# DannielSilva/MM-VQA

Measured on AMD Instinct MI355X. Metric: samples/sec ROCO-MLM pretrain (resnet152+transformer, bs16/GPU, 224^2, seq32), higher is better.
Workload: dtype f32; 1 GPU; pretrain/roco_train.py MLM-only: resnet152 + transformer(4 layers, 12 heads), num_vis 5, hidden 768, vocab 30522, per-GPU batch 16, 224x224, T=32; fwd + log_softmax/NLL + bwd + grad all-reduce + Adam; dropout on, train-mode BN; random-init weights; global_batch=16, seq_len=32, parallelism=dp1

## Files before the change

### mm-vqa_amd/csrc/common.h

```cpp
#pragma once
#include <hip/hip_runtime.h>
#include <stdint.h>
#include "../../include/mmvqa.h"

typedef float f32x4 __attribute__((ext_vector_type(4)));
typedef float f32x16 __attribute__((ext_vector_type(16)));

enum { ACT_NONE = 0, ACT_RELU = 1, ACT_GELU = 2, ACT_SERF = 3, ACT_SILU = 4, ACT_SIGMOID = 5 };
enum { PRO_NONE = 0, PRO_AFFINE_RELU = 1, PRO_DZ = 2, PRO_AFFINE = 3, PRO_AFFINE_SILU = 4, PRO_SILU_GATE = 5 };
enum { EPI_PLAIN = 0, EPI_TAP_FWD = 1, EPI_TAP_BWD = 2 };
enum { KIND_FWD = 0, KIND_DGRAD = 1, KIND_WGRAD = 2 };


typedef mmvqa_gemm_desc GemmParams;
typedef mmvqa_attn_desc AttnParams;

__device__ __forceinline__ float erf_pos(float s) {
  float t = 1.0f + s * (0.0705230784f + s * (0.0422820123f + s * (0.0092705272f +
            s * (0.0001520143f + s * (0.0002765672f + s * 0.0000430638f)))));
  t = t * t; t = t * t; t = t * t; t = t * t;
  const float big = 1.0f - 1.0f / t;
  const float s2 = s * s;
  float pl = -7.5757575757e-4f;
  pl = pl * s2 + 4.6296296296e-3f;
  pl = pl * s2 - 2.3809523810e-2f;
  pl = pl * s2 + 0.1f;
// ... 180 lines not shown
```

### mm-vqa_amd/csrc/elementwise.hip

```cpp
#include <cstring>

#include "common.h"

static inline int cdiv_i(long a, long b) { return (int)((a + b - 1) / b); }

static_assert(MMVQA_STAT_SLOTS == 16, "one lane per statistics replica");
__device__ __forceinline__ void stat_fold16(const double* __restrict__ stat, int C, int c, bool live, double& s0,
                                            double& s1) {
  typedef double f64x2 __attribute__((ext_vector_type(2)));
  const int sl = threadIdx.x & 15;
  f64x2 v = {0.0, 0.0};
  if (live) v = *reinterpret_cast<const f64x2*>(stat + ((size_t)sl * C + c) * 2);
  s0 = v[0]; s1 = v[1];
#pragma unroll
  for (int o = 8; o > 0; o >>= 1) { s0 += __shfl_xor(s0, o, 64); s1 += __shfl_xor(s1, o, 64); }
}
__global__ __launch_bounds__(256) void bn_coef_fwd_kernel(const double* __restrict__ stat, int C, double count, float eps,
                                   const float* __restrict__ gamma, const float* __restrict__ beta,
                                   float* __restrict__ run_mean, float* __restrict__ run_var,
                                   long long* __restrict__ nbt, double keep, int reps, int training,
                                   float* __restrict__ scale, float* __restrict__ shift,
                                   float* __restrict__ mean_out, float* __restrict__ invstd_out) {
  const int c = blockIdx.x * 16 + (threadIdx.x >> 4);
  if (blockIdx.x == 0 && threadIdx.x == 0 && training && nbt) *nbt += reps;
// ... 161 lines not shown
    double a[8] = {0, 0, 0, 0, 0, 0, 0, 0};
    for (int t = tid; t < 256; t += C4)
#pragma unroll
      for (int j = 0; j < 8; ++j) a[j] += red[t * 8 + j];
    int slot = blockIdx.x & (MMVQA_STAT_SLOTS - 1);
#pragma unroll
    for (int j = 0; j < 4; ++j) {
      double* d = stat + ((size_t)slot * C + tid * 4 + j) * 2;
      atomicAdd(d, a[j]);
      atomicAdd(d + 1, a[4 + j]);
    }
  }
}

#define LN_MAXV 4
__global__ void layernorm_fwd_kernel(const float* __restrict__ x, const float* __restrict__ res,
                                     const float* __restrict__ gamma, const float* __restrict__ beta,
                                     float* __restrict__ y, float* __restrict__ sum_out,
                                     float* __restrict__ mean_out, float* __restrict__ rstd_out,
                                     int rows, int H, float eps) {
  const int lane = threadIdx.x & 63;
  const int row = blockIdx.x * (blockDim.x >> 6) + (threadIdx.x >> 6);
  if (row >= rows) return;
  const int H4 = H / 4;
  f32x4 v[LN_MAXV];
  float s = 0.f;
#pragma unroll
  for (int j = 0; j < LN_MAXV; ++j) {
    int q = lane + 64 * j;
    v[j] = f32x4{0, 0, 0, 0};
// ... 21 lines not shown
  float rstd = 1.0f / sqrtf(var + eps);
#pragma unroll
  for (int j = 0; j < LN_MAXV; ++j) {
    int q = lane + 64 * j;
    if (q < H4) {
      f32x4 g = reinterpret_cast<const f32x4*>(gamma)[q], b = reinterpret_cast<const f32x4*>(beta)[q], o;
#pragma unroll
      for (int e = 0; e < 4; ++e) o[e] = (v[j][e] - mean) * rstd * g[e] + b[e];
      reinterpret_cast<f32x4*>(y + (size_t)row * H)[q] = o;
    }
  }
  if (lane == 0) { mean_out[row] = mean; rstd_out[row] = rstd; }
}

__global__ void layernorm_bwd_kernel(const float* __restrict__ dy, const float* __restrict__ x,
                                     const float* __restrict__ gamma, const float* __restrict__ mean,
                                     const float* __restrict__ rstd, const float* __restrict__ dres,
                                     float* __restrict__ dx, float* __restrict__ dgamma,
                                     float* __restrict__ dbeta, int rows, int H, int rows_per_wave) {
  extern __shared__ float lds[];
  const int lane = threadIdx.x & 63, wave = threadIdx.x >> 6, nw = blockDim.x >> 6;
  const int H4 = H / 4;
  for (int i = threadIdx.x; i < 2 * H; i += blockDim.x) lds[i] = 0.f;
  __syncthreads();
  f32x4 ag[LN_MAXV], ab[LN_MAXV];
#pragma unroll
  for (int j = 0; j < LN_MAXV; ++j) { ag[j] = f32x4{0, 0, 0, 0}; ab[j] = f32x4{0, 0, 0, 0}; }
  const int row0 = (blockIdx.x * nw + wave) * rows_per_wave;
  for (int rr = 0; rr < rows_per_wave; ++rr) {
    const int row = row0 + rr;
// ... 743 lines not shown
  }
  for (; i < n4; i += stride) {
    f32x4 p0 = P4[i], g0 = G4[i], m0 = M4[i], v0 = V4[i];
    upd(p0, g0, m0, v0);
    P4[i] = p0; M4[i] = m0; V4[i] = v0;
    if (zero_grad) G4[i] = zero;
  }
}

__global__ void axpy_kernel(float* __restrict__ y, const float* __restrict__ x, float a, long n) {
  long i = (long)blockIdx.x * blockDim.x + threadIdx.x;
  long stride = (long)gridDim.x * blockDim.x;
  for (; i < n; i += stride) y[i] += a * x[i];
}

__global__ void colsum_kernel(const float* __restrict__ x, int ld, int rows, int cols, float* __restrict__ out) {
  int c = blockIdx.x * blockDim.x + threadIdx.x;
  if (c >= cols) return;
  int r0 = blockIdx.y * 64, r1 = min(rows, r0 + 64);
  float s = 0.f;
  for (int r = r0; r < r1; ++r) s += x[(size_t)r * ld + c];
  atomicAdd(&out[c], s);
}

__global__ void dropout_kernel(float* __restrict__ x, long n, float p, uint32_t seed) {
  long i = (long)blockIdx.x * blockDim.x + threadIdx.x;
  long stride = (long)gridDim.x * blockDim.x;
  const float ks = 1.0f / (1.0f - p);
  for (; i < n; i += stride) x[i] = (rng_uniform(seed, (uint32_t)i) >= p) ? x[i] * ks : 0.f;
}

// ... 145 lines not shown
  return MMVQA_OK;
}

int k_layernorm_fwd(hipStream_t st, const float* x, const float* res, const float* gamma, const float* beta,
                    float* y, float* sum_out, float* mean, float* rstd, int rows, int H, float eps) {
  if (H % 4 != 0 || H > 256 * LN_MAXV) return mmvqa_set_error(MMVQA_ERR_ARG, "layernorm: H=%d unsupported", H);
  hipLaunchKernelGGL(layernorm_fwd_kernel, dim3(cdiv_i(rows, 4)), dim3(256), 0, st, x, res, gamma, beta, y,
                     sum_out, mean, rstd, rows, H, eps);
  KERNEL_CHECK_RET();
  return MMVQA_OK;
}

int k_layernorm_bwd(hipStream_t st, const float* dy, const float* x, const float* gamma, const float* mean,
                    const float* rstd, const float* dres, float* dx, float* dgamma, float* dbeta, int rows, int H) {
  if (H % 4 != 0 || H > 256 * LN_MAXV) return mmvqa_set_error(MMVQA_ERR_ARG, "layernorm: H=%d unsupported", H);
  int rpw = rows >= 2048 ? 4 : (rows >= 512 ? 2 : 1);
  int grid = cdiv_i(rows, 4 * rpw);
  hipLaunchKernelGGL(layernorm_bwd_kernel, dim3(grid), dim3(256), 2 * H * sizeof(float), st, dy, x, gamma, mean,
                     rstd, dres, dx, dgamma, dbeta, rows, H, rpw);
  KERNEL_CHECK_RET();
  return MMVQA_OK;
}

int k_embed_fwd(hipStream_t st, const long long* ids, const long long* seg, const float* word, const float* pos,
                const float* type, const float* gamma, const float* beta, const float* vis, float* out,
                float* xhat, float* rstd, int B, int T, int H, int num_vis, float eps, float drop_p,
                uint32_t seed) {
  if (H % 4 != 0 || H > 256 * LN_MAXV) return mmvqa_set_error(MMVQA_ERR_ARG, "embed: H=%d unsupported", H);
  hipLaunchKernelGGL(embed_fwd_kernel, dim3(cdiv_i((long)B * T, 4)), dim3(256), 0, st, ids, seg, word, pos, type,
                     gamma, beta, vis, out, xhat, rstd, B, T, H, num_vis, eps, drop_p, seed);
  KERNEL_CHECK_RET();
  return MMVQA_OK;
}

// ... 140 lines not shown
  hipLaunchKernelGGL(adam_kernel<U_>, dim3(grid_for(n / 4, 256, cap > 0 ? cap : 16384)), dim3(256), 0, st, p, g, m, v, n / 4, \
                     (float)(lr / bc1), (float)b1, (float)(1.0 - b1), (float)b2, (float)(1.0 - b2), (float)eps,            \
                     (float)sqrt(bc2), gscale, zero_grad)
  if (unroll >= 4) ADAM_GO(4); else if (unroll == 3) ADAM_GO(3); else if (unroll == 1) ADAM_GO(1); else ADAM_GO(2);
#undef ADAM_GO
  KERNEL_CHECK_RET();
  return MMVQA_OK;
}

int k_axpy(hipStream_t st, float* y, const float* x, float a, long n) {
  hipLaunchKernelGGL(axpy_kernel, dim3(grid_for(n)), dim3(256), 0, st, y, x, a, n);
  KERNEL_CHECK_RET();
  return MMVQA_OK;
}

int k_colsum(hipStream_t st, const float* x, int ld, int rows, int cols, float* out) {
  hipLaunchKernelGGL(colsum_kernel, dim3(cdiv_i(cols, 256), cdiv_i(rows, 64)), dim3(256), 0, st, x, ld, rows, cols,
                     out);
  KERNEL_CHECK_RET();
  return MMVQA_OK;
}

int k_dropout(hipStream_t st, float* x, long n, float p, uint32_t seed) {
  hipLaunchKernelGGL(dropout_kernel, dim3(grid_for(n)), dim3(256), 0, st, x, n, p, seed);
  KERNEL_CHECK_RET();
  return MMVQA_OK;
}

__global__ void pixmask_kernel(int* out, int total, int OH, int OW, int SH, int SW, int KH, int KW, int stride, int pad) {
  const int m = blockIdx.x * blockDim.x + threadIdx.x;
  if (m >= total) return;
  const int rem = m % (OH * OW), oy = rem / OW, ox = rem - oy * OW;
  const int y0 = oy * stride - pad, x0 = ox * stride - pad;
  unsigned mk = 0;
  for (int kh = 0; kh < KH; ++kh)
    for (int kw = 0; kw < KW; ++kw)
      if ((unsigned)(y0 + kh) < (unsigned)SH && (unsigned)(x0 + kw) < (unsigned)SW) mk |= 1u << (kh * KW + kw);
  out[m] = (int)mk;
}

int k_pixmask(hipStream_t st, int* out, int N, int OH, int OW, int SH, int SW, int KH, int KW, int stride, int pad) {
  if (KH * KW > 32) return mmvqa_set_error(MMVQA_ERR_ARG, "pixmask: at most 32 taps");
  const int total = N * OH * OW;
  if (total <= 0) return MMVQA_OK;
  hipLaunchKernelGGL(pixmask_kernel, dim3((total + 255) / 256), dim3(256), 0, st, out, total, OH, OW, SH, SW, KH, KW, stride, pad);
  KERNEL_CHECK_RET();
  return MMVQA_OK;
}

int k_dropout_copy(hipStream_t st, const float* x, float* y, long n, float p, uint32_t seed) {
  hipLaunchKernelGGL(dropout_copy_kernel, dim3(grid_for(n)), dim3(256), 0, st, x, y, n, p, seed);
  KERNEL_CHECK_RET();
  return MMVQA_OK;
}


__global__ void bn_act_add_kernel(const float* __restrict__ z, const float* __restrict__ s,
// ... 645 lines not shown
```

### mm-vqa_amd/csrc/engine.cpp

```cpp
#include "engine.h"

#include <cmath>
#include <cstdarg>
#include <cstdio>
#include <cstring>

static thread_local char g_err[1024] = "";
int mmvqa_set_error(int code, const char* fmt, ...) {
  va_list ap;
  va_start(ap, fmt);
  vsnprintf(g_err, sizeof(g_err), fmt, ap);
  va_end(ap);
  return code;
}
const char* mmvqa_get_error() { return g_err; }

#define TRY(x)                    \
  do {                            \
    int _r = (x);                 \
    if (_r != MMVQA_OK) return _r; \
  } while (0)

namespace {

// ... 211 lines not shown
  if (forced == 1 || forced == 2 || forced == 4 || forced == 8 || forced == 16) return forced;
  const double row_tiles = rows / 64.0;
  return row_tiles >= 32.0 ? 4 : (row_tiles >= 8.0 ? 2 : 1);
}

void plan_bn(Arena& a, BNRef& bn, double count) {
  bn.count = count;
  const size_t C = bn.C;
  bn.scale = a.f(C); bn.shift = a.f(C); bn.mean = a.f(C); bn.invstd = a.f(C);
  bn.P = a.f(C); bn.Q = a.f(C); bn.R = a.f(C);
}

}

static inline int conv_out(int x, int k, int s, int p) { return (x + 2 * p - k) / s + 1; }

size_t engine_plan(mmvqa_engine* e, int B, int T, int IH, int IW) {
  const mmvqa_model_desc& d = e->d;
  if (B <= 0 || T <= 0 || T > 128 || T > d.max_pos || T <= d.num_vis) {
    mmvqa_set_error(MMVQA_ERR_ARG, "plan: bad B=%d T=%d (max_pos %d, num_vis %d, T<=128)", B, T, d.max_pos, d.num_vis);
    return 0;
  }
  e->B = B; e->T = T; e->IH = IH; e->IW = IW;
  e->pixmask_off.clear(); e->ws_ready = false;
  Arena a;
  const int H = d.hidden;
  const size_t M = (size_t)B * T;
  size_t max_io = 0, max_mid = 0, max_tapM = 0;
  if (d.cnn == 1) {
    auto same = [](int in, int k, int s2, int* out) {
// ... 55 lines not shown
  e->SH = conv_out(IH, 7, 2, 3); e->SW = conv_out(IW, 7, 2, 3);
  e->PH = conv_out(e->SH, 3, 2, 1); e->PW = conv_out(e->SW, 3, 2, 1);
  const int w = d.resnet_width;
  const size_t M0 = (size_t)B * e->SH * e->SW;
  e->z0 = a.f(M0 * w);
  plan_bn(a, e->stem_bn, (double)M0);
  e->p0 = a.f((size_t)B * e->PH * e->PW * w);
  e->pool_idx = a.f(((size_t)B * e->PH * e->PW * w + 3) / 4);
  int h = e->PH, wd = e->PW;
  max_io = M0 * w; max_tapM = M0;
  for (auto& blk : e->blocks) {
    blk.N = B; blk.H = h; blk.W = wd;
    blk.OH = conv_out(h, 3, blk.c2.stride, 1); blk.OW = conv_out(wd, 3, blk.c2.stride, 1);
    const size_t Min = (size_t)B * h * wd, Mout = (size_t)B * blk.OH * blk.OW;
    blk.z1 = a.f(Min * blk.c1.Cout);
    if (blk.c2.stride == 1) {
      char key[96];
      snprintf(key, sizeof(key), "%d,%d,%d,%d,%d", B, blk.OH, blk.OW, blk.c2.KH, blk.c2.pad);
      if (!e->pixmask_off.count(key))
        e->pixmask_off[key] = mmvqa_engine::PixGeom{B, blk.OH, blk.OW, h, wd, blk.c2.KH, blk.c2.stride, blk.c2.pad, a.f(Mout)};
    }
    blk.z2 = a.f(Mout * blk.c2.Cout);
    blk.z3 = a.f(Mout * blk.c3.Cout);
    blk.out = a.f(Mout * blk.c3.Cout);
    plan_bn(a, blk.b1, (double)Min);
    plan_bn(a, blk.b2, (double)Mout);
    plan_bn(a, blk.b3, (double)Mout);
    if (blk.has_ds) { blk.zd = a.f(Mout * blk.cd.Cout); plan_bn(a, blk.bd, (double)Mout); }
    if (e->bn_fold) {
      blk.b1.slots = fold_slots((double)Min);
      blk.b2.slots = blk.b3.slots = blk.bd.slots = fold_slots((double)Mout);
    }
    max_io = std::max(max_io, std::max(Min * blk.c1.Cin, Mout * blk.c3.Cout));
    max_mid = std::max(max_mid, std::max(Min * blk.c1.Cout, Mout * blk.c2.Cout));
    h = blk.OH; wd = blk.OW;
  }
// ... 272 lines not shown
}

static int conv_wgrad(mmvqa_engine* e, hipStream_t st, const ConvRef& c, const float* G, const float* z,
                      const BNRef& bn_out, const float* x, const BNRef* bn_in, int N, int H, int W, int OH, int OW) {
  GemmParams g;
  memset(&g, 0, sizeof(g));
  g.M = c.Cout; g.N = c.KH * c.KH * c.Cin; g.K = N * OH * OW;
  g.A = G; g.A2 = z; g.a_ld = c.Cout; g.a_pro = PRO_DZ;
  g.a_c0 = WS(bn_out.P); g.a_c1 = WS(bn_out.Q); g.a_c2 = WS(bn_out.R);
  if (folding(e)) set_fold_bwd(e, g.a_fold, bn_out, false);
  g.B = x; g.b_ld = c.Cin;
  if (bn_in) { g.b_pro = PRO_AFFINE_RELU; g.b_c0 = WS(bn_in->scale); g.b_c1 = WS(bn_in->shift); }
  g.g_SH = H; g.g_SW = W; g.g_Cs = c.Cin; g.g_OH = OH; g.g_OW = OW;
  conv_geom(g, c, H, W, OH, OW);
  g.C = GRD(c.w); g.c_ld = g.N; g.c_atomic = 1;
  if (c.KH > 1 && c.stride == 1 && OH == H && OW == W) {
    char key[96];
    snprintf(key, sizeof(key), "%d,%d,%d,%d,%d", N, OH, OW, c.KH, c.pad);
    auto it = e->pixmask_off.find(key);
    if (it != e->pixmask_off.end()) g.pixmask = reinterpret_cast<int*>(WS(it->second.off));
  }
  RUN(PROF_IGEMM, 2.0 * (double)g.M * g.N * g.K, mmvqa_launch_igemm(g, KIND_WGRAD, 0, 0, st));
  return MMVQA_OK;
}

static int conv_dgrad(mmvqa_engine* e, hipStream_t st, const ConvRef& c, const float* G, const float* z,
                      const BNRef& bn_out, int N, int H, int W, int OH, int OW, float* dx, const EpiOpt& o) {
  GemmParams g;
  memset(&g, 0, sizeof(g));
  g.M = N * H * W; g.N = c.Cin; g.K = c.KH * c.KH * c.Cout;
  g.A = G; g.A2 = z; g.a_ld = c.Cout; g.a_pro = PRO_DZ;
  g.a_c0 = WS(bn_out.P); g.a_c1 = WS(bn_out.Q); g.a_c2 = WS(bn_out.R);
  if (folding(e)) set_fold_bwd(e, g.a_fold, bn_out, true);
  g.g_SH = OH; g.g_SW = OW; g.g_Cs = c.Cout; g.g_OH = H; g.g_OW = W;
// ... 1078 lines not shown
```

### mm-vqa_amd/csrc/igemm.hip

```cpp
#include <string>
#include <type_traits>
#include <vector>

#include "kernels.h"

struct FastDiv {
  uint32_t mul, shr, d;
};
struct GemmAux {
  FastDiv ohw, ow;
  int fast;
  int stagger;
  float* part;
  int ldsc;
  int sk_G;
  int sk_gx, sk_gy;
  int sk_slots;
  float* sk_part;
  unsigned* sk_cnt;
  int tick;
  int xcd;
};

__device__ __forceinline__ int fdiv(int n, const FastDiv& f) {
// ... 735 lines not shown
#pragma unroll
        for (int r = 0; r < NBC; ++r)
          f_voffB[r] = b_colvalid ? ((bkm_k0 + B_KSTEP * r) * p.b_ld + b_base[r]) * 4 : BIG;
      } else if constexpr (FAST == 1) {
        rB = __builtin_amdgcn_make_buffer_rsrc((void*)p.B, 0, p.K * p.b_ld * 4, FLAGS);
#pragma unroll
        for (int r = 0; r < NBC; ++r) f_voffB[r] = b_colvalid ? (b_base[r] * p.b_ld + b_ci) * 4 : BIG;
      } else {
        f_tapw = n0 / p.g_Cs;
        const int kh = f_tapw / p.g_KW, kw = f_tapw - kh * p.g_KW;
        rB = __builtin_amdgcn_make_buffer_rsrc((void*)(p.B - (p.g_pad * p.g_SW + p.g_pad) * p.b_ld), 0, NREC, FLAGS);
        rT = __builtin_amdgcn_make_buffer_rsrc((void*)p.pixmask, 0, p.K * 4, FLAGS);
        f_runB = (kh * p.g_SW + kw) * p.b_ld * 4;
#pragma unroll
        for (int r = 0; r < NBC; ++r) {
          f_voffB[r] = b_colvalid ? (b_base[r] * p.b_ld + b_ci) * 4 : BIG;
          f_voffT[r] = b_base[r] * 4;
        }
      }
#pragma unroll
      for (int r = 0; r < NBC; ++r) f_veB[r] = f_voffB[r];
    }
    int f_ve[NAC];
#pragma unroll
    for (int r = 0; r < NAC; ++r) f_ve[r] = (FAST != 0) ? f_voffA[r] : 0;
    auto tload = [&](int voff, int soff) __attribute__((always_inline)) {
      return __builtin_amdgcn_raw_buffer_load_b32(rT, voff, soff, 0);
    };
    auto f_halo = [&](Stage& S) __attribute__((always_inline)) {
      if constexpr (FAST == 2 && KIND == KIND_WGRAD) {
#pragma unroll
        for (int r = 0; r < NBC; ++r) {
          const int t = __builtin_amdgcn_sbfe(S.pm[r], f_tapw, 1);
          S.tmb[r] = t;
          f_veB[r] = (t & f_voffB[r]) | (~t & BIG);
          S.pm[r] = tload(f_voffT[r], f_runT + 2 * BK * 4);
        }
      } else if constexpr (FAST == 2) {
#pragma unroll
        for (int r = 0; r < NAC; ++r) {
          const int t = __builtin_amdgcn_sbfe((int)a_mask[r], f_tap & 31, 1);
          S.tm[r] = t;
          f_ve[r] = (t & f_voffA[r]) | (~t & BIG);
        }
      }
    };
    auto f_scalars = [&](Stage& S) __attribute__((always_inline)) {
      if constexpr (A_ROWK) {
        const bool live = f_tap < taps;
        const int toff = (KIND == KIND_FWD) ? (f_kh * p.g_SW + f_kw) * p.a_ld
// ... 23 lines not shown
      }
    };
    auto f_advance = [&]() __attribute__((always_inline)) {
#ifdef EXP_NOADVANCE
      return;
#endif
      if constexpr (A_ROWK) {
        f_c += BK;
        if (f_c >= p.g_Cs) {
          f_c = 0; ++f_tap; ++f_kw;
          if (f_kw == p.g_KW) { f_kw = 0; ++f_kh; }
        }
        f_runB += BK * 4;
      } else {
        f_runA += BK * p.a_ld * 4;
        f_runB += BK * p.b_ld * 4;
        f_runT += BK * 4;
      }
    };
    auto fload_piece = [&](Stage& S, int i) __attribute__((always_inline)) {
      if (i == 0) { f_halo(S); f_scalars(S); }
      else f_chunk(S, i - 1);
      if (i == NLP - 1) f_advance();
    };
    auto fstore_chunk = [&](Stage& S, int buf, int c) __attribute__((always_inline)) {
      float* as = As + buf * A_TILE;
      float* bs = Bs + buf * B_TILE;
      typedef float f32x2 __attribute__((ext_vector_type(2)));
      if (c < NAC) {
        const int r = c;
        f32x4 v = S.ra[r];
// ... 16 lines not shown
            const int tmask = S.tm[r];
            const i32x4 vi = __builtin_bit_cast(i32x4, v) & i32x4{tmask, tmask, tmask, tmask};
            v = __builtin_bit_cast(f32x4, vi);
          }
        }
        if constexpr (A_ROWK) {
          lds_put(as, (a_r0 + RSTEP * r) * LDK + a_kq, v);
        } else {
          lds_put(as, (akm_k0 + A_KSTEP * r) * LDA_KM + akm_x4 * 4, v);
        }
      } else {
        const int r = c - NAC;
        f32x4 v = S.rb[r];
        if constexpr (KIND == KIND_WGRAD && BPRO == PRO_AFFINE_RELU) {
          const f32x2 lo = __builtin_elementwise_fma(v.xy, bc0.xy, bc1.xy), hi = __builtin_elementwise_fma(v.zw, bc0.zw, bc1.zw);
          if constexpr (FAST == 2) {
            const float lim = __builtin_bit_cast(float, S.tmb[r] & 0x7f800000);
            v[0] = __builtin_amdgcn_fmed3f(lo[0], 0.f, lim); v[1] = __builtin_amdgcn_fmed3f(lo[1], 0.f, lim);
            v[2] = __builtin_amdgcn_fmed3f(hi[0], 0.f, lim); v[3] = __builtin_amdgcn_fmed3f(hi[1], 0.f, lim);
          } else {
            v[0] = fmaxf(lo[0], 0.f); v[1] = fmaxf(lo[1], 0.f); v[2] = fmaxf(hi[0], 0.f); v[3] = fmaxf(hi[1], 0.f);
          }
        }
        if constexpr (B_ROWK) {
          lds_put(bs, (b_r0 + RSTEP * r) * LDK + b_kq, v);
        } else {
          lds_put(bs, (bkm_k0 + B_KSTEP * r) * LDB_KM + bkm_x4 * 4, v);
        }
      }
    };
    auto LP = [&](Stage& S, int kt, int i) __attribute__((always_inline)) {
// ... 24 lines not shown
        } else {
#pragma unroll
          for (int j = 0; j < 4; ++j) fb[i][j] = bs[(kg * 8 + lh * 4 + j) * LDB_KM + wn0 + i * 32 + li];
        }
      }
    };

    constexpr int NC = NAC + NBC;
    constexpr int NKG = BK / 8 / KS;

    TRACE_MARK(1);
    Stage S0, S1;
    S0.a_ok = S0.b_ok = S1.a_ok = S1.b_ok = 0;
    S0.ac0 = S1.ac0 = ac0_i; S0.ac1 = S1.ac1 = ac1_i; S0.ac2 = S1.ac2 = ac2_i;

    if constexpr (FAST == 2 && KIND == KIND_WGRAD) {
#pragma unroll
      for (int r = 0; r < NBC; ++r) { S0.pm[r] = tload(f_voffT[r], 0); S1.pm[r] = tload(f_voffT[r], BK * 4); }
    }
    if (nkt > 0) {
      LT(S0, kt_begin);
      if constexpr (PIPE) LT(S1, kt_begin + 1);
#pragma unroll
      for (int c = 0; c < NC; ++c) SC(S0, 0, kt_begin, c);
      if constexpr (FAST != 0 && PIPE && !F16) f_halo(S0);
    }
    __builtin_amdgcn_s_waitcnt(0x0F70);
    __syncthreads();
    TRACE_MARK(2);

    if constexpr (F16) {
// ... 161 lines not shown
        for (int c = 0; c < NC; ++c) SC(S0, buf ^ 1, kt_begin + t + 1, c);
        __syncthreads();
      }
    }
  };

  {
    using I0 = std::integral_constant<int, PRO_NONE>;
    using I1 = std::integral_constant<int, PRO_AFFINE_RELU>;
    using I2 = std::integral_constant<int, PRO_DZ>;
    using I4 = std::integral_constant<int, F16 ? PRO_NONE : PRO_AFFINE_SILU>;
    using I5 = std::integral_constant<int, F16 ? PRO_NONE : PRO_SILU_GATE>;
    using G = std::integral_constant<int, 0>;
    using F1 = std::integral_constant<int, 1>;
    using F2 = std::integral_constant<int, 2>;
    using L0 = std::integral_constant<bool, false>;
    using L1 = std::integral_constant<bool, true>;
    if constexpr (NCHW) {
      if (KIND == KIND_WGRAD && p.a_pro == PRO_DZ) run(I2{}, I0{}, G{}, L0{}); else run(I0{}, I0{}, G{}, L0{});
    } else if constexpr (KIND == KIND_FWD) {
      if (x.fast == 1) {
        if (p.a_pro == PRO_AFFINE_RELU) { if (x.ldsc) run(I1{}, I0{}, F1{}, L1{}); else run(I1{}, I0{}, F1{}, L0{}); }
        else run(I0{}, I0{}, F1{}, L0{});
      } else if (x.fast == 2) {
        if (p.a_pro == PRO_AFFINE_RELU) { if (x.ldsc) run(I1{}, I0{}, F2{}, L1{}); else run(I1{}, I0{}, F2{}, L0{}); }
        else run(I0{}, I0{}, F2{}, L0{});
      } else {
        switch (p.a_pro) {
          case PRO_AFFINE_RELU: run(I1{}, I0{}, G{}, L0{}); break;
          case PRO_AFFINE_SILU: run(I4{}, I0{}, G{}, L0{}); break;
// ... 14 lines not shown
    } else {
      if (x.fast == 1) {
        if (p.a_pro == PRO_DZ) {
          if (p.b_pro == PRO_AFFINE_RELU) run(I2{}, I1{}, F1{}, L0{}); else run(I2{}, I0{}, F1{}, L0{});
        } else {
          if (p.b_pro == PRO_AFFINE_RELU) run(I0{}, I1{}, F1{}, L0{}); else run(I0{}, I0{}, F1{}, L0{});
        }
      } else if (x.fast == 2) {
        if constexpr (TM * TN == 1) {
          if (p.a_pro == PRO_DZ) {
            if (p.b_pro == PRO_AFFINE_RELU) run(I2{}, I1{}, F2{}, L0{}); else run(I2{}, I0{}, F2{}, L0{});
          } else {
            if (p.b_pro == PRO_AFFINE_RELU) run(I0{}, I1{}, F2{}, L0{}); else run(I0{}, I0{}, F2{}, L0{});
          }
        }
      } else if (p.a_pro == PRO_DZ) {
        switch (p.b_pro) {
          case PRO_AFFINE_RELU: run(I2{}, I1{}, G{}, L0{}); break;
          case PRO_AFFINE_SILU: run(I2{}, I4{}, G{}, L0{}); break;
          case PRO_SILU_GATE: run(I2{}, I5{}, G{}, L0{}); break;
          default: run(I2{}, I0{}, G{}, L0{});
        }
      } else {
        switch (p.b_pro) {
          case PRO_AFFINE_RELU: run(I0{}, I1{}, G{}, L0{}); break;
          case PRO_AFFINE_SILU: run(I0{}, I4{}, G{}, L0{}); break;
          case PRO_SILU_GATE: run(I0{}, I5{}, G{}, L0{}); break;
          default: run(I0{}, I0{}, G{}, L0{});
        }
      }
// ... 254 lines not shown
  constexpr size_t epi_floats = (size_t)BM * (BN + 4) + 8 * BN;
  constexpr size_t smem_max = (tile_floats + FOLD_MAX_FLOATS > epi_floats ? tile_floats + FOLD_MAX_FLOATS : epi_floats) * sizeof(float);
  static int attr_dev_mask = 0;
  int dev = 0;
  (void)hipGetDevice(&dev);
  if (!(attr_dev_mask >> (dev & 31) & 1)) {
    HIP_CHECK_RET(hipFuncSetAttribute((const void*)igemm_kernel<BM, BN, BK, KIND, NCHW, KS, false, PREC>,
                                      hipFuncAttributeMaxDynamicSharedMemorySize, (int)smem_max));
    attr_dev_mask |= 1 << (dev & 31);
  }
  GemmAux x;
  x.ohw = make_fastdiv(p.g_OH * p.g_OW);
  x.ow = make_fastdiv(p.g_OW);
  x.fast = 0;
  static const int stagger_on = getenv("MMVQA_IGEMM_NOSTAGGER") ? 0 : 1;
  x.stagger = stagger_on;
  x.part = (KIND != KIND_WGRAD && !NCHW && p.splitk > 1 && !p.c_atomic) ? p.sk_ws : nullptr;
  if (!NCHW && (p.K % BK == 0 || (KIND == KIND_WGRAD && p.pixmask)) && !p.gate && !getenv("MMVQA_IGEMM_GENERAL")) {
    const int taps = p.g_KH * p.g_KW;
    const double lim = 2147483648.0 - 16777216.0;
    if (KIND != KIND_WGRAD) {
      const bool pro_ok = (KIND == KIND_FWD) ? (p.a_pro == PRO_NONE || p.a_pro == PRO_AFFINE_RELU)
                                             : (p.a_pro == PRO_NONE || p.a_pro == PRO_DZ);
      const double a_bytes = (KIND == KIND_FWD) ? (double)p.M * p.g_stride * p.g_stride * p.a_ld * 4.0 + (double)(p.g_SW + 2) * p.g_KH * p.a_ld * 4.0
                                                : (double)p.M * p.a_ld * 4.0;
      const double b_bytes = (KIND == KIND_FWD) ? (double)p.N * p.b_ld * 4.0 : (double)p.g_Cs * p.b_ld * 4.0;
      if (pro_ok && p.b_pro == PRO_NONE && p.g_Cs % BK == 0 && p.g_stride <= 2 && a_bytes < lim && b_bytes < lim &&
          (KIND == KIND_FWD || p.N % 4 == 0))
        x.fast = (taps > 1 || (KIND == KIND_DGRAD && p.g_stride > 1)) ? 2 : 1;
    } else {
      const bool pro_ok = (p.a_pro == PRO_NONE || p.a_pro == PRO_DZ) && (p.b_pro == PRO_NONE || p.b_pro == PRO_AFFINE_RELU);
      if (pro_ok && taps == 1 && p.K % BK == 0 && p.g_stride == 1 && p.g_pad == 0 && p.M % 4 == 0 && p.N % 4 == 0 &&
          (double)p.K * p.a_ld * 4.0 < lim && (double)p.K * p.b_ld * 4.0 < lim)
        x.fast = 1;
      else if (pro_ok && taps > 1 && taps <= 32 && p.pixmask && p.g_stride == 1 && p.g_OH == p.g_SH && p.g_OW == p.g_SW &&
               2 * p.g_pad == p.g_KH - 1 && p.g_KH == p.g_KW && BM == 64 && BN == 64 && p.g_Cs % BN == 0 && p.M % 4 == 0 &&
               (double)p.K * p.a_ld * 4.0 < lim && (double)(p.K + (double)p.g_SW * p.g_KH) * p.b_ld * 4.0 < lim)
        x.fast = 2;
    }
  }
  x.ldsc = 0;
  size_t fold_floats = 0;
  if (p.a_fold.stat) {
    const int ncoef = p.a_fold.bwd ? 3 : 2;
    const size_t need = A_ROWK ? (size_t)ncoef * p.g_Cs : (size_t)3 * BM;
    const bool pro_ok = p.a_fold.bwd ? p.a_pro == PRO_DZ : p.a_pro == PRO_AFFINE_RELU;
    if (pro_ok && need <= FOLD_MAX_FLOATS && (KIND == KIND_WGRAD || x.fast != 0)) {
      x.ldsc = 1;
      fold_floats = need;
    } else {
      const BnFold f = p.a_fold;
      const int C = A_ROWK ? p.g_Cs : p.M;
      if (!f.publish || !f.out0 || !f.out1 || !f.out2)
// ... 306 lines not shown
```

Measured before the change: 661.2 samples/s.

## Add strided wgrad source-map fast path, restructure LayerNorm bwd and colsum kernels

```diff
diff --git a/mm-vqa_amd/csrc/common.h b/mm-vqa_amd/csrc/common.h
--- a/mm-vqa_amd/csrc/common.h
+++ b/mm-vqa_amd/csrc/common.h
@@ -10,6 +10,7 @@
 enum { PRO_NONE = 0, PRO_AFFINE_RELU = 1, PRO_DZ = 2, PRO_AFFINE = 3, PRO_AFFINE_SILU = 4, PRO_SILU_GATE = 5 };
 enum { EPI_PLAIN = 0, EPI_TAP_FWD = 1, EPI_TAP_BWD = 2 };
 enum { KIND_FWD = 0, KIND_DGRAD = 1, KIND_WGRAD = 2 };
+#define PIX_SRC_SHIFT 9
 
 
 typedef mmvqa_gemm_desc GemmParams;
diff --git a/mm-vqa_amd/csrc/elementwise.hip b/mm-vqa_amd/csrc/elementwise.hip
--- a/mm-vqa_amd/csrc/elementwise.hip
+++ b/mm-vqa_amd/csrc/elementwise.hip
@@ -199,6 +199,8 @@
 }
 
 #define LN_MAXV 4
+#define LNB_WGS 256
+#define COLSUM_WGS 256
 __global__ void layernorm_fwd_kernel(const float* __restrict__ x, const float* __restrict__ res,
                                      const float* __restrict__ gamma, const float* __restrict__ beta,
                                      float* __restrict__ y, float* __restrict__ sum_out,
@@ -250,6 +252,84 @@
 }
 
 __global__ void layernorm_bwd_kernel(const float* __restrict__ dy, const float* __restrict__ x,
+                                     const float* __restrict__ gamma, const float* __restrict__ mean,
+                                     const float* __restrict__ rstd, const float* __restrict__ dres,
+                                     float* __restrict__ dx, float* __restrict__ dgamma,
+                                     float* __restrict__ dbeta, int rows, int H, int rows_per_wave) {
+  extern __shared__ float lds[];
+  const int lane = threadIdx.x & 63, wave = threadIdx.x >> 6, nw = blockDim.x >> 6;
+  const int H4 = H / 4;
+  f32x4 ag[LN_MAXV], ab[LN_MAXV], g[LN_MAXV];
+#pragma unroll
+  for (int j = 0; j < LN_MAXV; ++j) {
+    int q = lane + 64 * j;
+    ag[j] = f32x4{0, 0, 0, 0}; ab[j] = f32x4{0, 0, 0, 0}; g[j] = f32x4{0, 0, 0, 0};
+    if (q < H4) g[j] = reinterpret_cast<const f32x4*>(gamma)[q];
+  }
+  const int row0 = (blockIdx.x * nw + wave) * rows_per_wave;
+  for (int rr = 0; rr < rows_per_wave; ++rr) {
+    const int row = row0 + rr;
+    if (row >= rows) break;
+    f32x4 xh[LN_MAXV], dg[LN_MAXV], rv[LN_MAXV];
+#pragma unroll
+    for (int j = 0; j < LN_MAXV; ++j) {
+      int q = lane + 64 * j;
+      xh[j] = f32x4{0, 0, 0, 0}; dg[j] = f32x4{0, 0, 0, 0}; rv[j] = f32x4{0, 0, 0, 0};
+      if (q < H4) {
+        xh[j] = reinterpret_cast<const f32x4*>(x + (size_t)row * H)[q];
+        dg[j] = reinterpret_cast<const f32x4*>(dy + (size_t)row * H)[q];
+        if (dres) rv[j] = reinterpret_cast<const f32x4*>(dres + (size_t)row * H)[q];
+      }
+    }
+    const float mu = mean[row], rs = rstd[row];
+    float s1 = 0.f, s2 = 0.f;
+#pragma unroll
+    for (int j = 0; j < LN_MAXV; ++j) {
+      if (lane + 64 * j < H4) {
+#pragma unroll
+        for (int e = 0; e < 4; ++e) {
+          const float d = dg[j][e];
+          xh[j][e] = (xh[j][e] - mu) * rs;
+          dg[j][e] = d * g[j][e];
+          s1 += dg[j][e];
+          s2 += dg[j][e] * xh[j][e];
+          ag[j][e] += d * xh[j][e];
+          ab[j][e] += d;
+        }
+      }
+    }
+    s1 = wave_sum(s1) / (float)H;
+    s2 = wave_sum(s2) / (float)H;
+#pragma unroll
+    for (int j = 0; j < LN_MAXV; ++j) {
+      int q = lane + 64 * j;
+      if (q < H4) {
+        f32x4 o;
+#pragma unroll
+        for (int e = 0; e < 4; ++e) o[e] = rs * (dg[j][e] - s1 - xh[j][e] * s2) + rv[j][e];
+        reinterpret_cast<f32x4*>(dx + (size_t)row * H)[q] = o;
+      }
+    }
+  }
+  if (!dgamma) return;
+  float* slab = lds + (size_t)wave * 2 * H;
+#pragma unroll
+  for (int j = 0; j < LN_MAXV; ++j) {
+    int q = lane + 64 * j;
+    if (q < H4) {
+      reinterpret_cast<f32x4*>(slab)[q] = ag[j];
+      reinterpret_cast<f32x4*>(slab + H)[q] = ab[j];
+    }
+  }
+  __syncthreads();
+  for (int i = threadIdx.x; i < 2 * H; i += blockDim.x) {
+    float s = 0.f;
+    for (int w = 0; w < nw; ++w) s += lds[(size_t)w * 2 * H + i];
+    atomicAdd(i < H ? &dgamma[i] : &dbeta[i - H], s);
+  }
+}
+
+__global__ void layernorm_bwd_v0_kernel(const float* __restrict__ dy, const float* __restrict__ x,
                                      const float* __restrict__ gamma, const float* __restrict__ mean,
                                      const float* __restrict__ rstd, const float* __restrict__ dres,
                                      float* __restrict__ dx, float* __restrict__ dgamma,
@@ -1023,7 +1103,59 @@
   for (; i < n; i += stride) y[i] += a * x[i];
 }
 
-__global__ void colsum_kernel(const float* __restrict__ x, int ld, int rows, int cols, float* __restrict__ out) {
+template <int VEC, int U>
+__global__ __launch_bounds__(256) void colsum_kernel(const float* __restrict__ x, int ld, int rows, int cols,
+                                                     float* __restrict__ out) {
+  constexpr int CG = 128 / VEC, RS = 256 / CG;
+  __shared__ float red[RS][128];
+  const int cg = threadIdx.x % CG, rs = threadIdx.x / CG;
+  const long c = (long)blockIdx.x * 128 + cg * VEC;
+  const bool whole = c + VEC <= cols;
+  float acc[VEC];
+#pragma unroll
+  for (int e = 0; e < VEC; ++e) acc[e] = 0.f;
+  for (long rb = (long)blockIdx.y * (RS * U); rb < rows; rb += (long)gridDim.y * (RS * U)) {
+    float v[U][VEC];
+#pragma unroll
+    for (int u = 0; u < U; ++u) {
+      const long r = rb + rs + u * RS;
+      const float* src = x + (size_t)r * ld + c;
+#pragma unroll
+      for (int e = 0; e < VEC; ++e) v[u][e] = 0.f;
+      if (r < rows) {
+        if constexpr (VEC == 4) {
+          if (whole) {
+            f32x4 t = *reinterpret_cast<const f32x4*>(src);
+#pragma unroll
+            for (int e = 0; e < 4; ++e) v[u][e] = t[e];
+          } else {
+#pragma unroll
+            for (int e = 0; e < 4; ++e)
+              if (c + e < cols) v[u][e] = src[e];
+          }
+        } else {
+          if (whole) v[u][0] = src[0];
+        }
+      }
+    }
+#pragma unroll
+    for (int u = 0; u < U; ++u)
+#pragma unroll
+      for (int e = 0; e < VEC; ++e) acc[e] += v[u][e];
+  }
+#pragma unroll
+  for (int e = 0; e < VEC; ++e) red[rs][cg * VEC + e] = acc[e];
+  __syncthreads();
+  if (threadIdx.x < 128) {
+    const long oc = (long)blockIdx.x * 128 + threadIdx.x;
+    float s = 0.f;
+#pragma unroll
+    for (int k = 0; k < RS; ++k) s += red[k][threadIdx.x];
+    if (oc < cols) atomicAdd(&out[oc], s);
+  }
+}
+
+__global__ void colsum_v0_kernel(const float* __restrict__ x, int ld, int rows, int cols, float* __restrict__ out) {
   int c = blockIdx.x * blockDim.x + threadIdx.x;
   if (c >= cols) return;
   int r0 = blockIdx.y * 64, r1 = min(rows, r0 + 64);
@@ -1199,10 +1331,18 @@
 int k_layernorm_bwd(hipStream_t st, const float* dy, const float* x, const float* gamma, const float* mean,
                     const float* rstd, const float* dres, float* dx, float* dgamma, float* dbeta, int rows, int H) {
   if (H % 4 != 0 || H > 256 * LN_MAXV) return mmvqa_set_error(MMVQA_ERR_ARG, "layernorm: H=%d unsupported", H);
-  int rpw = rows >= 2048 ? 4 : (rows >= 512 ? 2 : 1);
-  int grid = cdiv_i(rows, 4 * rpw);
-  hipLaunchKernelGGL(layernorm_bwd_kernel, dim3(grid), dim3(256), 2 * H * sizeof(float), st, dy, x, gamma, mean,
-                     rstd, dres, dx, dgamma, dbeta, rows, H, rpw);
+  static const bool split_off = getenv("MMVQA_NO_LNB_SPLIT") != nullptr;
+  if (split_off) {
+    int rpw = rows >= 2048 ? 4 : (rows >= 512 ? 2 : 1);
+    hipLaunchKernelGGL(layernorm_bwd_v0_kernel, dim3(cdiv_i(rows, 4 * rpw)), dim3(256), 2 * H * sizeof(float), st, dy, x,
+                       gamma, mean, rstd, dres, dx, dgamma, dbeta, rows, H, rpw);
+    KERNEL_CHECK_RET();
+    return MMVQA_OK;
+  }
+  const int nw = rows > 2 * LNB_WGS ? 4 : 2;
+  const int rpw = cdiv_i(rows, (long)nw * LNB_WGS);
+  hipLaunchKernelGGL(layernorm_bwd_kernel, dim3(cdiv_i(rows, nw * rpw)), dim3(64 * nw), (size_t)nw * 2 * H * sizeof(float),
+                     st, dy, x, gamma, mean, rstd, dres, dx, dgamma, dbeta, rows, H, rpw);
   KERNEL_CHECK_RET();
   return MMVQA_OK;
 }
@@ -1373,9 +1513,31 @@
   return MMVQA_OK;
 }
 
+template <int VEC>
+static void colsum_launch(hipStream_t st, const float* x, int ld, int rows, int cols, float* out) {
+  constexpr int RS = 256 / (128 / VEC);
+  const int cb = cdiv_i(cols, 128);
+  int u = 8;
+  while (u > 1 && (long)cb * cdiv_i(rows, RS * u) < COLSUM_WGS) u >>= 1;
+  const dim3 grid(cb, std::min(cdiv_i(rows, RS * u), 65535)), block(256);
+  switch (u) {
+    case 8: hipLaunchKernelGGL((colsum_kernel<VEC, 8>), grid, block, 0, st, x, ld, rows, cols, out); break;
+    case 4: hipLaunchKernelGGL((colsum_kernel<VEC, 4>), grid, block, 0, st, x, ld, rows, cols, out); break;
+    case 2: hipLaunchKernelGGL((colsum_kernel<VEC, 2>), grid, block, 0, st, x, ld, rows, cols, out); break;
+    default: hipLaunchKernelGGL((colsum_kernel<VEC, 1>), grid, block, 0, st, x, ld, rows, cols, out); break;
+  }
+}
+
 int k_colsum(hipStream_t st, const float* x, int ld, int rows, int cols, float* out) {
-  hipLaunchKernelGGL(colsum_kernel, dim3(cdiv_i(cols, 256), cdiv_i(rows, 64)), dim3(256), 0, st, x, ld, rows, cols,
-                     out);
+  static const bool split_off = getenv("MMVQA_NO_COLSUM_SPLIT") != nullptr;
+  if (rows <= 0 || cols <= 0) return MMVQA_OK;
+  if (split_off)
+    hipLaunchKernelGGL(colsum_v0_kernel, dim3(cdiv_i(cols, 256), cdiv_i(rows, 64)), dim3(256), 0, st, x, ld, rows, cols,
+                       out);
+  else if (ld % 4 == 0 && ((uintptr_t)x & 15) == 0)
+    colsum_launch<4>(st, x, ld, rows, cols, out);
+  else
+    colsum_launch<1>(st, x, ld, rows, cols, out);
   KERNEL_CHECK_RET();
   return MMVQA_OK;
 }
@@ -1395,11 +1557,15 @@
   for (int kh = 0; kh < KH; ++kh)
     for (int kw = 0; kw < KW; ++kw)
       if ((unsigned)(y0 + kh) < (unsigned)SH && (unsigned)(x0 + kw) < (unsigned)SW) mk |= 1u << (kh * KW + kw);
+  if (stride > 1) mk |= (unsigned)((m / (OH * OW) * SH + oy * stride) * SW + ox * stride) << PIX_SRC_SHIFT;
   out[m] = (int)mk;
 }
 
 int k_pixmask(hipStream_t st, int* out, int N, int OH, int OW, int SH, int SW, int KH, int KW, int stride, int pad) {
   if (KH * KW > 32) return mmvqa_set_error(MMVQA_ERR_ARG, "pixmask: at most 32 taps");
+  if (stride > 1 && (KH * KW > PIX_SRC_SHIFT || (double)N * SH * SW + (double)pad * (SW + 1) > (double)(1 << (32 - PIX_SRC_SHIFT))))
+    return mmvqa_set_error(MMVQA_ERR_ARG, "pixmask: a strided geometry takes at most %d taps and 2^%d source pixels", PIX_SRC_SHIFT,
+                           32 - PIX_SRC_SHIFT);
   const int total = N * OH * OW;
   if (total <= 0) return MMVQA_OK;
   hipLaunchKernelGGL(pixmask_kernel, dim3((total + 255) / 256), dim3(256), 0, st, out, total, OH, OW, SH, SW, KH, KW, stride, pad);
diff --git a/mm-vqa_amd/csrc/engine.cpp b/mm-vqa_amd/csrc/engine.cpp
--- a/mm-vqa_amd/csrc/engine.cpp
+++ b/mm-vqa_amd/csrc/engine.cpp
@@ -249,6 +249,11 @@
 }
 
 static inline int conv_out(int x, int k, int s, int p) { return (x + 2 * p - k) / s + 1; }
+static std::string pix_key(int N, int H, int W, int OH, int OW, const ConvRef& c) {
+  char key[96];
+  snprintf(key, sizeof(key), "%d,%d,%d,%d,%d,%d,%d,%d", N, H, W, OH, OW, c.KH, c.stride, c.pad);
+  return key;
+}
 
 size_t engine_plan(mmvqa_engine* e, int B, int T, int IH, int IW) {
   const mmvqa_model_desc& d = e->d;
@@ -334,12 +339,14 @@
     blk.OH = conv_out(h, 3, blk.c2.stride, 1); blk.OW = conv_out(wd, 3, blk.c2.stride, 1);
     const size_t Min = (size_t)B * h * wd, Mout = (size_t)B * blk.OH * blk.OW;
     blk.z1 = a.f(Min * blk.c1.Cout);
-    if (blk.c2.stride == 1) {
-      char key[96];
-      snprintf(key, sizeof(key), "%d,%d,%d,%d,%d", B, blk.OH, blk.OW, blk.c2.KH, blk.c2.pad);
+    auto plan_pix = [&](const ConvRef& c) {
+      if (c.stride > 2 || (c.stride == 2 && (double)B * h * wd + (double)c.pad * (wd + 1) > (double)(1 << (32 - PIX_SRC_SHIFT)))) return;
+      const std::string key = pix_key(B, h, wd, blk.OH, blk.OW, c);
       if (!e->pixmask_off.count(key))
-        e->pixmask_off[key] = mmvqa_engine::PixGeom{B, blk.OH, blk.OW, h, wd, blk.c2.KH, blk.c2.stride, blk.c2.pad, a.f(Mout)};
-    }
+        e->pixmask_off[key] = mmvqa_engine::PixGeom{B, blk.OH, blk.OW, h, wd, c.KH, c.stride, c.pad, a.f(Mout)};
+    };
+    plan_pix(blk.c2);
+    if (blk.has_ds && blk.cd.stride == 2) plan_pix(blk.cd);
     blk.z2 = a.f(Mout * blk.c2.Cout);
     blk.z3 = a.f(Mout * blk.c3.Cout);
     blk.out = a.f(Mout * blk.c3.Cout);
@@ -642,10 +649,8 @@
   g.g_SH = H; g.g_SW = W; g.g_Cs = c.Cin; g.g_OH = OH; g.g_OW = OW;
   conv_geom(g, c, H, W, OH, OW);
   g.C = GRD(c.w); g.c_ld = g.N; g.c_atomic = 1;
-  if (c.KH > 1 && c.stride == 1 && OH == H && OW == W) {
-    char key[96];
-    snprintf(key, sizeof(key), "%d,%d,%d,%d,%d", N, OH, OW, c.KH, c.pad);
-    auto it = e->pixmask_off.find(key);
+  if ((c.KH > 1 && c.stride == 1 && OH == H && OW == W) || c.stride == 2) {
+    auto it = e->pixmask_off.find(pix_key(N, H, W, OH, OW, c));
     if (it != e->pixmask_off.end()) g.pixmask = reinterpret_cast<int*>(WS(it->second.off));
   }
   RUN(PROF_IGEMM, 2.0 * (double)g.M * g.N * g.K, mmvqa_launch_igemm(g, KIND_WGRAD, 0, 0, st));
diff --git a/mm-vqa_amd/csrc/igemm.hip b/mm-vqa_amd/csrc/igemm.hip
--- a/mm-vqa_amd/csrc/igemm.hip
+++ b/mm-vqa_amd/csrc/igemm.hip
@@ -773,7 +773,8 @@
         f_runB = (kh * p.g_SW + kw) * p.b_ld * 4;
 #pragma unroll
         for (int r = 0; r < NBC; ++r) {
-          f_voffB[r] = b_colvalid ? (b_base[r] * p.b_ld + b_ci) * 4 : BIG;
+          if constexpr (FAST == 3) f_voffB[r] = b_colvalid ? b_ci * 4 : BIG;
+          else f_voffB[r] = b_colvalid ? (b_base[r] * p.b_ld + b_ci) * 4 : BIG;
           f_voffT[r] = b_base[r] * 4;
         }
       }
@@ -787,12 +788,14 @@
       return __builtin_amdgcn_raw_buffer_load_b32(rT, voff, soff, 0);
     };
     auto f_halo = [&](Stage& S) __attribute__((always_inline)) {
-      if constexpr (FAST == 2 && KIND == KIND_WGRAD) {
+      if constexpr (FAST >= 2 && KIND == KIND_WGRAD) {
+        const int ldb4 = p.b_ld * 4;
 #pragma unroll
         for (int r = 0; r < NBC; ++r) {
           const int t = __builtin_amdgcn_sbfe(S.pm[r], f_tapw, 1);
           S.tmb[r] = t;
-          f_veB[r] = (t & f_voffB[r]) | (~t & BIG);
+          const int off = (FAST == 3) ? (int)((unsigned)S.pm[r] >> PIX_SRC_SHIFT) * ldb4 + f_voffB[r] : f_voffB[r];
+          f_veB[r] = (t & off) | (~t & BIG);
           S.pm[r] = tload(f_voffT[r], f_runT + 2 * BK * 4);
         }
       } else if constexpr (FAST == 2) {
@@ -846,7 +849,7 @@
         f_runB += BK * 4;
       } else {
         f_runA += BK * p.a_ld * 4;
-        f_runB += BK * p.b_ld * 4;
+        if constexpr (FAST != 3) f_runB += BK * p.b_ld * 4;
         f_runT += BK * 4;
       }
     };
@@ -893,7 +896,7 @@
         f32x4 v = S.rb[r];
         if constexpr (KIND == KIND_WGRAD && BPRO == PRO_AFFINE_RELU) {
           const f32x2 lo = __builtin_elementwise_fma(v.xy, bc0.xy, bc1.xy), hi = __builtin_elementwise_fma(v.zw, bc0.zw, bc1.zw);
-          if constexpr (FAST == 2) {
+          if constexpr (FAST >= 2) {
             const float lim = __builtin_bit_cast(float, S.tmb[r] & 0x7f800000);
             v[0] = __builtin_amdgcn_fmed3f(lo[0], 0.f, lim); v[1] = __builtin_amdgcn_fmed3f(lo[1], 0.f, lim);
             v[2] = __builtin_amdgcn_fmed3f(hi[0], 0.f, lim); v[3] = __builtin_amdgcn_fmed3f(hi[1], 0.f, lim);
@@ -948,7 +951,7 @@
     S0.a_ok = S0.b_ok = S1.a_ok = S1.b_ok = 0;
     S0.ac0 = S1.ac0 = ac0_i; S0.ac1 = S1.ac1 = ac1_i; S0.ac2 = S1.ac2 = ac2_i;
 
-    if constexpr (FAST == 2 && KIND == KIND_WGRAD) {
+    if constexpr (FAST >= 2 && KIND == KIND_WGRAD) {
 #pragma unroll
       for (int r = 0; r < NBC; ++r) { S0.pm[r] = tload(f_voffT[r], 0); S1.pm[r] = tload(f_voffT[r], BK * 4); }
     }
@@ -1140,6 +1143,7 @@
     using G = std::integral_constant<int, 0>;
     using F1 = std::integral_constant<int, 1>;
     using F2 = std::integral_constant<int, 2>;
+    using F3 = std::integral_constant<int, 3>;
     using L0 = std::integral_constant<bool, false>;
     using L1 = std::integral_constant<bool, true>;
     if constexpr (NCHW) {
@@ -1184,6 +1188,14 @@
             if (p.b_pro == PRO_AFFINE_RELU) run(I0{}, I1{}, F2{}, L0{}); else run(I0{}, I0{}, F2{}, L0{});
           }
         }
+      } else if (x.fast == 3) {
+        if constexpr (TM * TN == 1 && !F16) {
+          if (p.a_pro == PRO_DZ) {
+            if (p.b_pro == PRO_AFFINE_RELU) run(I2{}, I1{}, F3{}, L0{}); else run(I2{}, I0{}, F3{}, L0{});
+          } else {
+            if (p.b_pro == PRO_AFFINE_RELU) run(I0{}, I1{}, F3{}, L0{}); else run(I0{}, I0{}, F3{}, L0{});
+          }
+        }
       } else if (p.a_pro == PRO_DZ) {
         switch (p.b_pro) {
           case PRO_AFFINE_RELU: run(I2{}, I1{}, G{}, L0{}); break;
@@ -1468,6 +1480,7 @@
   x.ow = make_fastdiv(p.g_OW);
   x.fast = 0;
   static const int stagger_on = getenv("MMVQA_IGEMM_NOSTAGGER") ? 0 : 1;
+  const bool srcmap_off = getenv("MMVQA_NO_WGRAD_SRCMAP") != nullptr;
   x.stagger = stagger_on;
   x.part = (KIND != KIND_WGRAD && !NCHW && p.splitk > 1 && !p.c_atomic) ? p.sk_ws : nullptr;
   if (!NCHW && (p.K % BK == 0 || (KIND == KIND_WGRAD && p.pixmask)) && !p.gate && !getenv("MMVQA_IGEMM_GENERAL")) {
@@ -1491,6 +1504,14 @@
                2 * p.g_pad == p.g_KH - 1 && p.g_KH == p.g_KW && BM == 64 && BN == 64 && p.g_Cs % BN == 0 && p.M % 4 == 0 &&
                (double)p.K * p.a_ld * 4.0 < lim && (double)(p.K + (double)p.g_SW * p.g_KH) * p.b_ld * 4.0 < lim)
         x.fast = 2;
+      else if (pro_ok && PREC == MMVQA_PREC_F32 && p.pixmask && p.g_stride == 2 && p.g_KH == p.g_KW &&
+               ((taps == 9 && p.g_pad == 1) || (taps == 1 && p.g_pad == 0)) && BM == 64 && BN == 64 &&
+               (taps == 1 || p.g_Cs % BN == 0) && p.M % 4 == 0 && p.N % 4 == 0 && !srcmap_off) {
+        const double src_n = (double)(p.K / (p.g_OH * p.g_OW)) * p.g_SH * p.g_SW + (double)p.g_pad * (p.g_SW + 1);
+        if (src_n <= (double)(1 << (32 - PIX_SRC_SHIFT)) && (double)p.K * p.a_ld * 4.0 < lim &&
+            (src_n + (double)p.g_SW * p.g_KH) * p.b_ld * 4.0 < lim)
+          x.fast = 3;
+      }
     }
   }
   x.ldsc = 0;
```

Result: no change. 663.0 samples/s, median of 6 (+0.3%).
